# watsonyanghx/GAN_Lib_Tensorflow

Hardware: AMD Instinct MI355X
Metric: images/sec (G+D step) SNGAN-ResNet CIFAR-10 bs=64 (higher is better)
Workload: dtype bf16; 1 GPU; SNGAN ResNet CIFAR-10 32x32 bs=64 hinge: 1 G update (2x64 fakes) + 5 D updates (64 real + 64 fake) per step; global_batch=64, per_gpu_batch=64, parallelism=dp1, graphs=True, finite=True, collectives_in_graphs=False, grad_wire=fp32

## Files before the change

### gan_lib_tensorflow_amd/_lib.py

```python
import ctypes as C
import os

_HERE = os.path.dirname(os.path.abspath(__file__))
DTYPE = os.environ.get("GANK_DTYPE", "bf16").lower()
if DTYPE not in ("bf16", "fp16"):
    raise RuntimeError(f"GANK_DTYPE={DTYPE!r}: bf16 or fp16")
ACT_DTYPE_NAME = "bfloat16" if DTYPE == "bf16" else "float16"
LIB_PATH = os.path.join(_HERE, os.environ.get("GANK_LIB_NAME", "libgank.so" if DTYPE == "bf16" else "libgank_f16.so"))

P, I, L, F = C.c_void_p, C.c_int, C.c_long, C.c_float

IN_UPSAMPLE2X, IN_RELU, OUT_TANH, DY_UPSAMPLE2X, RES_UPSAMPLE2X, STATS_PREZEROED, OUT_POOLSUM2X = 1, 2, 4, 8, 64, 256, 512
STAT_SLOTS = 16


class SnDesc(C.Structure):
    _fields_ = [(n, P) for n in ("W", "u_in", "u_out", "v", "W_bar", "scal", "a", "b", "bpart",
                                 "dW_bar", "dW", "rowdot", "ga", "u_snap")] + \
               [("K", I), ("C", I), ("row_offset", I), ("chunk_offset", I)]


class WgradItem(C.Structure):
    _fields_ = [("x", P), ("dy", P), ("dw", P), ("dbias", P)]

# ... 8 lines not shown

class Res8Head(C.Structure):
    _fields_ = [("logits", P), ("head_w", P), ("pooled", P), ("loss", P), ("w_grad", P), ("b_grad", P), ("n_real", I), ("mode", I),
                ("loss_scale", F)]


class LabelDenseDesc(C.Structure):
    _fields_ = [("table", P), ("bias", P), ("out", P), ("V", I), ("D", I), ("weight", I)]


class CriticFeedDesc(C.Structure):
    _fields_ = [("real_all", P), ("labels_all", P), ("fake_all", P), ("both", P), ("labels2", P), ("slot", P), ("rng_state", P),
                ("done_counter", P), ("B", I), ("n_slots", I)]


PROTOTYPES = {
    "gank_version": [],
    "gank_act_dtype": [],
    "gank_last_error": [],
    "gank_conv2d_prep_weights": [P, P, P, I, I, I, P],
    "gank_conv2d_prep_weights_batched": [C.POINTER(PrepDesc), I, P],
    "gank_conv2d_fprop": [P, P, P, P, P, P, I, I, I, I, I, I, I, F, P],
    "gank_conv2d_fprop_stats": [P, P, P, P, P, P, I, I, I, I, I, I, I, F, P, I, P, P],
    "gank_conv2d_dgrad": [P, P, P, P, P, I, I, I, I, I, I, I, F, P],
    "gank_meanpool_conv1x1_fprop": [P, P, P, P, P, I, I, I, I, I, P],
    "gank_image_conv_pair_fprop": [P, P, P, P, P, P, P, P, I, I, I, I, I, P],
    "gank_conv2d_wgrad_batched": [C.POINTER(WgradItem), I, I, I, I, I, I, I, I, F, P],
    "gank_conv2d_wgrad_narrow_pair": [P, P, P, P, I, I, I, I, I, P, P, P, P, I, I, I, I, I, F, P],
    "gank_conv2d_wgrad_ws_elems": [I, I, I, I, I, I, I],
    "gank_conv1x1_wgrad_dgrad": [P, P, P, P, P, I, P, I, I, I, I, I, P],
    "gank_conv2d_wgrad": [P, P, P, P, P, L, I, I, I, I, I, I, I, F, P],
    "gank_upconv3x3_prep_weights": [P, P, P, I, I, P],
    "gank_upconv3x3_fprop": [P, P, P, P, P, I, I, I, I, I, I, P],
    "gank_upconv3x3_fprop_stats": [P, P, P, P, P, I, I, I, I, I, I, P, I, P, P],
    "gank_upconv3x3_dgrad": [P, P, P, P, I, I, I, I, I, P],
    "gank_convpool3x3_prep_weights": [P, P, P, I, I, P],
    "gank_convpool3x3_fprop": [P, P, P, P, P, I, I, I, I, I, I, P],
    "gank_convpool3x3_dgrad": [P, P, P, P, I, I, I, I, I, P],
    "gank_convpool3x3_wgrad": [P, P, P, P, P, L, I, I, I, I, I, I, P],
    "gank_convpool3x3_wgrad_ws_elems": [I, I, I, I, I],
    "gank_upconv3x3_wgrad_ws_elems": [I, I, I, I, I],
    "gank_upconv3x3_wgrad": [P, P, P, P, L, I, I, I, I, I, P],
    "gank_conv2d_general_fprop": [P, P, P, P, I, I, I, I, I, I, I, I, I, I, I, P],
    "gank_conv2d_general_dgrad": [P, P, P, P, I, I, I, I, I, I, I, I, I, P],
    "gank_conv2d_general_wgrad": [P, P, P, P, I, I, I, I, I, I, I, I, I, I, I, P],
    "gank_res8_chain_fwd": [P, P, P, P, P, P, I, I, I, P],
    "gank_res8_chain_bwd": [P, P, P, P, P, P, P, P, P, I, I, I, P],
    "gank_phase_stack4": [P, P, I, I, I, P],
    "gank_pad_rows": [P, P, C.c_long, I, I, I, I, P],
    "gank_tile_rows": [P, P, I, I, I, P],
    "gank_fewout_pack": [P, P, I, I, I, I, I, P],
    "gank_zero_f32": [P, C.c_long, P],
    "gank_img16_conv3x3": [P, P, P, P, P, P, I, I, I, I, P],
    "gank_cbn_relu_img16_conv3x3": [P, P, P, P, P, P, P, P, P, I, I, I, I, I, I, P, I, P],
    "gank_img16_conv3x3_stats": [P, P, P, P, P, P, I, I, I, I, P, I, P],
    "gank_res8_chain_fwd_head": [P, P, P, P, P, P, P, P, P, I, I, I, P],
    "gank_res8_chain_bwd_head": [C.POINTER(Res8Head), P, P, P, P, P, P, P, I, I, I, P],
    "gank_res8_conv3x3": [P, P, P, P, P, I, I, I, I, P, I, P],
    "gank_im2col_narrow": [P, P, I, I, I, I, I, I, I, I, I, I, P],
    "gank_tap_gather_up2": [P, P, P, I, I, I, I, I, I, I, I, P],
    "gank_tap_scatter_up2": [P, P, I, I, I, I, I, I, I, P],
    "gank_depth_to_space2": [P, P, I, I, I, I, P],
    "gank_space_to_depth2": [P, P, I, I, I, I, P],
    "gank_cpool_res_fprop": [P, P, P, P, P, I, I, I, I, I, I, P],
    "gank_cpool_res_dgrad": [P, P, P, P, I, I, I, I, I, P],
    "gank_cpool_res_dgrad_image_wgrad": [P, P, P, P, P, P, P, P, P, I, I, I, I, I, P, P],
# ... 161 lines not shown
```

### gan_lib_tensorflow_amd/csrc/conv_igemm.hip

```cpp
#include "gank_common.h"
#ifdef GANK_TUNING
static __device__ int gank_stats_dbg = 0;
static void gank_stats_dbg_init() {
  static const int v = gank_tune("GANK_STATS_DBG", 0);
  static bool done = false;
  if (!done) { done = true; if (v) (void)hipMemcpyToSymbol(HIP_SYMBOL(gank_stats_dbg), &v, sizeof(int)); }
}
#else
static inline void gank_stats_dbg_init() {}
#endif
#include <stdlib.h>
#include <type_traits>

#ifndef GANK_KMODE
#define GANK_KMODE 0
#endif
#define IG_IN_ZEROINS2X 16
#define IG_IN_STRIDE2 32
#define IG_RES_UP2X 128

struct IgemmArgs {
  const bf16* x;
  const bf16* w;
  const float* bias;
// ... 991 lines not shown
  gank_prof_tag(0, tag.c_str());
  hipLaunchKernelGGL((conv_narrow_in_kernel<KS, CIN, POOL>), dim3(a.tiles_m * a.tiles_n), dim3(256), 0, s, a);
  GANK_LAUNCH_OK("conv_narrow_in");
  return 0;
}

constexpr int PP_HALO_BYTES = 24576;
constexpr int PP_WSLOT_BYTES = 16384;
constexpr int PP_NSLOT = 6, PP_PD = 4;
constexpr int PP_WRING = 2 * PP_HALO_BYTES;
constexpr int PP_LDS_BYTES = PP_WRING + PP_NSLOT * PP_WSLOT_BYTES;

template <int N>
__device__ __forceinline__ void pp_wait_vmcnt() {
  static_assert(N == 0 || N == 4 || N == 6 || N == 7, "vmcnt value not instantiated");
  if constexpr (N == 0) asm volatile("s_waitcnt vmcnt(0)" ::: "memory");
  if constexpr (N == 4) asm volatile("s_waitcnt vmcnt(4)" ::: "memory");
  if constexpr (N == 6) asm volatile("s_waitcnt vmcnt(6)" ::: "memory");
  if constexpr (N == 7) asm volatile("s_waitcnt vmcnt(7)" ::: "memory");
}

#ifndef GANK_PP_M16
#define GANK_PP_M16 1
#endif
#ifdef GANK_ACT_F16
#define GANK_MFMA16(a, b, c) __builtin_amdgcn_mfma_f32_16x16x32_f16(a, b, c, 0, 0, 0)
#else
#define GANK_MFMA16(a, b, c) __builtin_amdgcn_mfma_f32_16x16x32_bf16(a, b, c, 0, 0, 0)
#endif
template <int MODE, int PW, bool STATS = false>
__global__ __launch_bounds__(512) void conv_igemm_pp_kernel(IgemmArgs a) {
  constexpr bool PHASE = (MODE & 4) != 0;
  constexpr int NT = PHASE ? 4 : 9;
  constexpr int PHH = 256 / PW;
  constexpr int HW_ = PW + 2, HROW = HW_ * 64;
  constexpr int HPX = (PHH + 2) * HW_;
  constexpr int RS = 32 / PW;
  constexpr int HSW = PW == 16 ? 1 : 2;
#if GANK_PP_M16
  auto pp_hswz = [](int hx) { return (hx >> 1) & 2; };
  auto pp_wswz = [](int co) { return (co >> 1) & 2; };
#else
  auto pp_hswz = [](int hx) { return (hx >> HSW) & 3; };
  auto pp_wswz = [](int co) { return (co >> 2) & 3; };
#endif
  static_assert(PW == 32 || PW == 16, "patch width");
  static_assert(HPX * 64 <= PP_HALO_BYTES, "halo image");
  extern __shared__ __attribute__((aligned(16))) char smem[];
  typedef __attribute__((address_space(3))) void* lds_t;
  const int tid = threadIdx.x, lane = tid & 63;
  const int wave = __builtin_amdgcn_readfirstlane(tid >> 6);
  const int wm = wave >> 2, wn = wave & 3;
  const int r = lane & 31, h = lane >> 5;
  const int prow = RS == 1 ? 0 : (r >> 4), pcol = RS == 1 ? r : (r & 15);

  const int nwg = a.tiles_m * a.tiles_n;
  const int lid = xcd_remap(blockIdx.x, nwg);
  const int tile_n = lid % a.tiles_n;
  int tile_m = lid / a.tiles_n;
  int phase = 0;
  if constexpr (PHASE) {
    if (a.phase_inner) { phase = tile_m & 3; tile_m >>= 2; }
    else { phase = tile_m / a.tiles_pp; tile_m -= phase * a.tiles_pp; }
  }
  const int pad_h = PHASE ? 1 - (phase >> 1) : 1, pad_w = PHASE ? 1 - (phase & 1) : 1;
  const int pw = a.W / PW, ph = a.H / PHH;
  const int n = tile_m / (pw * ph), pr = tile_m - n * pw * ph;
  const int py0 = (pr / pw) * PHH, px0 = (pr % pw) * PW;

  constexpr unsigned OOB = 0x7FFFFFF0u;
  const __amdgpu_buffer_rsrc_t rs_x = __builtin_amdgcn_make_buffer_rsrc(const_cast<bf16*>(a.x), 0, a.N * a.H * a.W * a.Cin * 2, 0x00020000);
  const __amdgpu_buffer_rsrc_t rs_w = __builtin_amdgcn_make_buffer_rsrc(const_cast<bf16*>(a.w) + (PHASE ? (long)phase * a.CoutPad * a.Kpad : 0L), 0,
                                                                        a.CoutPad * a.Kpad * 2, 0x00020000);

  unsigned h_off[6];
#pragma unroll
  for (int j = 0; j < 6; j++) {
    const int q = (j * 4 + wn) * 64 + lane;
    const int hp = q >> 2, hy = hp / HW_, hx = hp - hy * HW_;
    const int iy = py0 - 1 + hy, ix = px0 - 1 + hx;
    const bool ok = hp < HPX && (unsigned)iy < (unsigned)a.H && (unsigned)ix < (unsigned)a.W;
    h_off[j] = ok ? (unsigned)((((n * a.H + iy) * a.W + ix) * a.Cin + (((q & 3) ^ pp_hswz(hx)) << 3)) * 2) : OOB;
  }
  int w_off[2];
#pragma unroll
  for (int j = 0; j < 2; j++) {
    const int q = (j * 8 + wave) * 64 + lane;
    const int co = q >> 2;
    w_off[j] = ((tile_n * 256 + co) * a.Kpad + (((q & 3) ^ pp_wswz(co)) << 3)) * 2;
  }
  constexpr int ND = PHASE ? 2 : 3;
#if GANK_PP_M16
  const int p16 = lane & 15, kc = lane >> 4;
  constexpr int RPT = PW / 16;
  int a_lane, b_lane[ND];
  a_lane = PP_WRING + (wn * 64 + p16) * 64 + ((kc ^ pp_wswz(p16)) << 4);
#pragma unroll
  for (int d = 0; d < ND; d++) {
    const int hx = p16 + d + (PHASE ? 1 - pad_w : 0);
    const int hy = wm * (PHH / 2) + (PHASE ? 1 - pad_h : 0);
    b_lane[d] = hy * HROW + hx * 64 + ((kc ^ pp_hswz(hx)) << 4);
  }
#else
  int a_lane[2], b_lane[ND][2];
#pragma unroll
  for (int kk = 0; kk < 2; kk++) {
    a_lane[kk] = PP_WRING + (wn * 64 + r) * 64 + (((kk * 2 + h) ^ pp_wswz(r)) << 4);
#pragma unroll
    for (int d = 0; d < ND; d++) {
      const int hx = pcol + d + (PHASE ? 1 - pad_w : 0);
      const int hy = wm * (PHH / 2) + prow + (PHASE ? 1 - pad_h : 0);
      b_lane[d][kk] = hy * HROW + hx * 64 + (((kk * 2 + h) ^ pp_hswz(hx)) << 4);
    }
  }
#endif

  const int nch = a.Cin >> 5;
  auto issue_w = [&](int slot_bytes, int c, int tap) {
    const int koff = (tap * a.Cin + c * 32) * 2;
#pragma unroll
    for (int j = 0; j < 2; j++)
      __builtin_amdgcn_raw_ptr_buffer_load_lds(rs_w, (lds_t)(smem + PP_WRING + slot_bytes + (j * 8 + wave) * 1024), 16, w_off[j], koff, 0, 0);
  };
  auto issue_h = [&](int buf, int c, int j0) {
#pragma unroll
    for (int j = j0; j < j0 + 3; j++)
      __builtin_amdgcn_raw_ptr_buffer_load_lds(rs_x, (lds_t)(smem + buf * PP_HALO_BYTES + (j * 4 + wn) * 1024), 16, (int)(h_off[j] + (unsigned)c * 64u), 0, 0, 0);
  };

#if GANK_PP_M16
  f32x4 acc[4][8];
#pragma unroll
  for (int i = 0; i < 4; i++)
#pragma unroll
    for (int j = 0; j < 8; j++) acc[i][j] = f32x4{0.f, 0.f, 0.f, 0.f};
#else
  f32x16 acc[2][4];
#pragma unroll
  for (int i = 0; i < 2; i++)
#pragma unroll
    for (int j = 0; j < 4; j++)
#pragma unroll
      for (int e = 0; e < 16; e++) acc[i][j][e] = 0.f;
#endif

  if (wm == 1) { issue_h(0, 0, 0); issue_h(0, 0, 3); }
  {
    int c = 0, t = 0;
#pragma unroll
    for (int q = 0; q < PP_PD; q++) {
      issue_w(q * PP_WSLOT_BYTES, c, t);
      if (++t == NT) { t = 0; c++; }
      if (c >= nch) { c = nch - 1; t = NT - 1; }
    }
  }
  pp_wait_vmcnt<4>();
  __builtin_amdgcn_s_barrier();

  int rslot = 0, wslot = PP_PD * PP_WSLOT_BYTES;
  for (int c = 0; c < nch; c++) {
    const int hb = (c & 1) * PP_HALO_BYTES;
    const int cn = (c + 1 < nch) ? c + 1 : nch - 1;
    auto phase_step = [&](auto tc) {
      constexpr int t = decltype(tc)::value;
      constexpr int dh1 = PHASE ? t / 2 : t / 3, dw1 = PHASE ? t % 2 : t % 3;
      if (wm == 1) __builtin_amdgcn_s_barrier();
#if GANK_PP_M16
      bf16x8 fa[4], fb[8];
#pragma unroll
      for (int i = 0; i < 4; i++) fa[i] = *reinterpret_cast<const bf16x8*>(smem + rslot + i * 1024 + a_lane);
#pragma unroll
      for (int j = 0; j < 8; j++) fb[j] = *reinterpret_cast<const bf16x8*>(smem + hb + (j / RPT + dh1) * HROW + (j % RPT) * 1024 + b_lane[dw1]);
#else
      bf16x8 fa[2][2], fb[4][2];
#pragma unroll
      for (int kk = 0; kk < 2; kk++) {
#pragma unroll
        for (int i = 0; i < 2; i++) fa[i][kk] = *reinterpret_cast<const bf16x8*>(smem + rslot + i * 2048 + a_lane[kk]);
#pragma unroll
        for (int j = 0; j < 4; j++) fb[j][kk] = *reinterpret_cast<const bf16x8*>(smem + hb + (j * RS + dh1) * HROW + b_lane[dw1][kk]);
      }
#endif
      if constexpr (t < 2) { if (wm == 1) issue_h((c + 1) & 1, cn, 3 * t); }
      {
        constexpr int t4 = (t + PP_PD) % NT;
        int c4 = c + (t + PP_PD) / NT, tt = t4;
        if (c4 >= nch) { c4 = nch - 1; tt = NT - 1; }
        issue_w(wslot, c4, tt);
      }
      if constexpr (t < 2) { if (wm == 1) pp_wait_vmcnt<7>(); else pp_wait_vmcnt<4>(); }
      else pp_wait_vmcnt<4>();
      if (wm == 0) __builtin_amdgcn_s_barrier();
      asm volatile("s_waitcnt lgkmcnt(0)" ::: "memory");
#if GANK_PP_M16
      if constexpr ((MODE & 1) != 0) {
#pragma unroll
        for (int j = 0; j < 8; j++) fb[j] = __builtin_bit_cast(bf16x8, relu_bf16x8(__builtin_bit_cast(u32x4, fb[j])));
      }
      __builtin_amdgcn_sched_barrier(0);
#pragma unroll
      for (int i = 0; i < 4; i++)
#pragma unroll
        for (int j = 0; j < 8; j++)
          acc[i][j] = GANK_MFMA16(fa[i], fb[j], acc[i][j]);
#else
      if constexpr ((MODE & 1) != 0) {
#pragma unroll
        for (int j = 0; j < 4; j++)
#pragma unroll
          for (int kk = 0; kk < 2; kk++) fb[j][kk] = __builtin_bit_cast(bf16x8, relu_bf16x8(__builtin_bit_cast(u32x4, fb[j][kk])));
      }
      __builtin_amdgcn_sched_barrier(0);
#pragma unroll
      for (int kk = 0; kk < 2; kk++)
#pragma unroll
        for (int i = 0; i < 2; i++)
#pragma unroll
          for (int j = 0; j < 4; j++)
            acc[i][j] = GANK_MFMA32(fa[i][kk], fb[j][kk], acc[i][j]);
#endif
      __builtin_amdgcn_sched_barrier(0);
      rslot += PP_WSLOT_BYTES; if (rslot == PP_NSLOT * PP_WSLOT_BYTES) rslot = 0;
      wslot += PP_WSLOT_BYTES; if (wslot == PP_NSLOT * PP_WSLOT_BYTES) wslot = 0;
    };
    phase_step(std::integral_constant<int, 0>{}); phase_step(std::integral_constant<int, 1>{});
    phase_step(std::integral_constant<int, 2>{}); phase_step(std::integral_constant<int, 3>{});
    if constexpr (!PHASE) {
      phase_step(std::integral_constant<int, 4>{}); phase_step(std::integral_constant<int, 5>{}); phase_step(std::integral_constant<int, 6>{});
      phase_step(std::integral_constant<int, 7>{}); phase_step(std::integral_constant<int, 8>{});
    }
  }
  pp_wait_vmcnt<0>();

  const bool otanh = (a.flags & GANK_OUT_TANH) != 0;
  float keep1 = 0.f, keep2 = 0.f;
#if GANK_PP_M16
  {
    float st1[STATS ? 2 : 1][8], st2[STATS ? 2 : 1][8];
    if constexpr (STATS) {
#pragma unroll
      for (int P = 0; P < 2; P++)
#pragma unroll
        for (int e = 0; e < 8; e++) { st1[P][e] = 0.f; st2[P][e] = 0.f; }
    }
#pragma unroll
    for (int j = 0; j < 8; j++) {
      const int py = py0 + wm * (PHH / 2) + j / RPT, px = px0 + (j % RPT) * 16 + p16;
      const long m = PHASE ? ((long)(n * 2 * a.H + 2 * py + (phase >> 1))) * (2 * a.W) + 2 * px + (phase & 1) : ((long)(n * a.H + py)) * a.W + px;
      const long mr = (!PHASE && (a.flags & IG_RES_UP2X)) ? ((long)(n * (a.H >> 1) + (py >> 1))) * (a.W >> 1) + (px >> 1) : m;
      bf16x8 outl[2];
#pragma unroll
      for (int P = 0; P < 2; P++) {
        const int co = tile_n * 256 + wn * 64 + (2 * P + (kc & 1)) * 16 + 8 * (kc >> 1);
        float v[8];
#pragma unroll
        for (int e = 0; e < 4; e++) {
          float lo = acc[2 * P][j][e] * a.scale, hi = acc[2 * P + 1][j][e] * a.scale;
          asm volatile("s_nop 1\n\tv_permlane16_swap_b32 %0, %1" : "+v"(lo), "+v"(hi));
          v[e] = lo;
          v[4 + e] = hi;
        }
        const long o = m * a.Cout + co;
        float bb[8] = {0.f, 0.f, 0.f, 0.f, 0.f, 0.f, 0.f, 0.f}, d[8];
        if (a.bias) {
          const f32x4 b0 = *reinterpret_cast<const f32x4*>(a.bias + co), b1 = *reinterpret_cast<const f32x4*>(a.bias + co + 4);
#pragma unroll
          for (int e = 0; e < 4; e++) { bb[e] = b0[e]; bb[4 + e] = b1[e]; }
        }
#pragma unroll
        for (int e = 0; e < 8; e++) { d[e] = v[e]; v[e] += bb[e]; }
        if (a.mask) {
          const bf16x8 mk = *reinterpret_cast<const bf16x8*>(a.mask + o);
#pragma unroll
          for (int e = 0; e < 8; e++) { const bool on = bf2f(mk[e]) > 0.f; v[e] = on ? v[e] : 0.f; d[e] = on ? d[e] : -bb[e]; }
        }
        if (a.res) {
          const bf16x8 rs = *reinterpret_cast<const bf16x8*>(a.res + mr * a.Cout + co);
#pragma unroll
          for (int e = 0; e < 8; e++) { const float t = bf2f(rs[e]); v[e] += t; d[e] += t; }
        }
        if constexpr (STATS) {
#pragma unroll
          for (int e = 0; e < 8; e++) { st1[P][e] += d[e]; st2[P][e] += d[e] * d[e]; }
        }
#pragma unroll
        for (int e = 0; e < 8; e++) outl[P][e] = f2bf(otanh ? tanhf(v[e]) : v[e]);
      }
      bf16* line = a.y + m * a.Cout + tile_n * 256 + wn * 64 + (kc & 1) * 16 + 8 * (kc >> 1);
#pragma unroll
      for (int P = 0; P < 2; P++) *reinterpret_cast<bf16x8*>(line + 32 * P) = outl[P];
    }
    if constexpr (STATS) {
#pragma unroll
      for (int P = 0; P < 2; P++)
#pragma unroll
        for (int e = 0; e < 8; e++) {
          const float s1 = pp_row_sum(st1[P][e]), s2 = pp_row_sum(st2[P][e]);
          const bool mine = p16 == P * 8 + e;
          keep1 = mine ? s1 : keep1;
          keep2 = mine ? s2 : keep2;
        }
    }
  }
  if constexpr (STATS) {
    float* dst = a.stat_sums + ((long)(n / a.stat_n_per_group) * GANK_STAT_SLOTS + (blockIdx.x % GANK_STAT_SLOTS)) * 2 * a.Cout;
    const int co = tile_n * 256 + wn * 64 + (2 * (p16 >> 3) + (kc & 1)) * 16 + 8 * (kc >> 1) + (p16 & 7);
#ifdef GANK_TUNING
    if (gank_stats_dbg) return;
#endif
    atomicAdd(dst + co, keep1);
    atomicAdd(dst + a.Cout + co, keep2);
  }
#else
  {
    float st1[STATS ? 2 : 1][2][8], st2[STATS ? 2 : 1][2][8];
    if constexpr (STATS) {
#pragma unroll
      for (int i = 0; i < 2; i++)
#pragma unroll
        for (int q = 0; q < 2; q++)
#pragma unroll
          for (int e = 0; e < 8; e++) { st1[i][q][e] = 0.f; st2[i][q][e] = 0.f; }
    }
// ... 70 lines not shown
    const int ci = r >> 4, cq = (r >> 3) & 1, ce = r & 7;
    const int co = tile_n * 256 + (wn * 2 + ci) * 32 + 16 * cq + 8 * h + ce;
#ifdef GANK_TUNING
    if (gank_stats_dbg) return;
#endif
    atomicAdd(dst + co, keep1);
    atomicAdd(dst + a.Cout + co, keep2);
  }
#endif
}

static thread_local int tl_stats_done = 0;
__global__ void ig_zero_kernel(float* __restrict__ p, int n) {
  const int i = blockIdx.x * blockDim.x + threadIdx.x;
  if (i < n) p[i] = 0.f;
}

static void stats_zero(const IgemmArgs& a, hipStream_t s);
static int t128_min() {
  static const int v = gank_tune("GANK_IGEMM_T128_MIN", 192);
  return v;
}
static bool igemm_stats_ok(const IgemmArgs& a, int BM, int BN) {
  static const int env = gank_tune("GANK_IGEMM_STATS", 1);
  return env && a.stat_sums != nullptr && !(a.flags & GANK_OUT_TANH) && a.M % BM == 0 && a.Cout % BN == 0 &&
         ((long)a.stat_n_per_group * a.H * a.W) % BM == 0;
}
template <int MODE, int PW>
static int launch_pp(const IgemmArgs& a0, hipStream_t s) {
  IgemmArgs a = a0;
  const bool stats = a.stat_sums != nullptr;
  if (stats) { tl_stats_done = 1; stats_zero(a, s); }
  constexpr bool PHASE = (MODE & 4) != 0;
  const int tiles = a.N * (a.H / (256 / PW)) * (a.W / PW);
  a.tiles_pp = tiles;
  a.phase_inner = phase_inner_env();
  a.tiles_m = PHASE ? 4 * tiles : tiles;
  a.tiles_n = a.Cout / 256;
  if (PHASE) { a.Kpad = 4 * a.Cin; a.Hin = a.H; a.Win = a.W; }
  auto kern = stats ? conv_igemm_pp_kernel<MODE, PW, true> : conv_igemm_pp_kernel<MODE, PW, false>;
  if (stats) { GANK_MAX_DYNAMIC_LDS((conv_igemm_pp_kernel<MODE, PW, true>), PP_LDS_BYTES, "conv_igemm_pp"); }
  else { GANK_MAX_DYNAMIC_LDS((conv_igemm_pp_kernel<MODE, PW, false>), PP_LDS_BYTES, "conv_igemm_pp"); }
  static const std::string tag = gank_format("conv_igemm_pp_kernel<%d, %d>", MODE, PW);
  gank_prof_tag(0, tag.c_str());
  hipLaunchKernelGGL(kern, dim3(a.tiles_m * a.tiles_n), dim3(512), PP_LDS_BYTES, s, a);
  GANK_LAUNCH_OK("conv_igemm_pp");
  return 0;
}
static int pp_patch_width(int H, int W) { return (W % 32 == 0 && H % 8 == 0) ? 32 : (W % 16 == 0 && H % 16 == 0) ? 16 : 0; }
static int pp_env() {
  static const int v = gank_tune("GANK_IGEMM_PP", 2);
  return v;
}
static bool pp_enough_blocks(const IgemmArgs& a, int phases) {
  const int pw = pp_patch_width(a.H, a.W);
  return pw != 0 && (long)phases * a.N * (a.H / (256 / pw)) * (a.W / pw) * (a.Cout / 256) >= 224;
}
static bool pp_phase_ok(const IgemmArgs& a) {
  return pp_env() >= 2 && a.Cout % 256 == 0 && a.Cin % 32 == 0 && pp_enough_blocks(a, 4);
}
static int launch_pp_phase(const IgemmArgs& a, hipStream_t s) {
  const bool relu = (a.flags & GANK_IN_RELU) != 0;
  if (pp_patch_width(a.H, a.W) == 32) return relu ? launch_pp<5, 32>(a, s) : launch_pp<4, 32>(a, s);
  return relu ? launch_pp<5, 16>(a, s) : launch_pp<4, 16>(a, s);
}

template <int MODE, int BN>
static int launch_patch(const IgemmArgs& a0, hipStream_t s) {
  IgemmArgs a = a0;
  a.tiles_m = a.N * (a.H / 8) * (a.W / 16);
  a.tiles_n = a.CoutPad / BN;
  const size_t lds = ((size_t)10 * HROWP + (size_t)2 * BN * LROW) * sizeof(bf16);
  auto kern = conv_igemm_patch_kernel<MODE, BN>;
  GANK_MAX_DYNAMIC_LDS(kern, (int)lds, "conv_igemm_patch");
  static const std::string tag = gank_format("conv_igemm_patch_kernel<%d, %d>", MODE, BN);
  gank_prof_tag(0, tag.c_str());
  hipLaunchKernelGGL(kern, dim3(a.tiles_m * a.tiles_n), dim3(256), lds, s, a);
  GANK_LAUNCH_OK("conv_igemm_patch");
  return 0;
}

template <int WM, int WN, int TM, int TN, bool PACKED, int PF, int MODE>
static int launch_cfg(const IgemmArgs& a0, hipStream_t s) {
  IgemmArgs a = a0;
  constexpr int BM = WM * TM * 32, BN = WN * TN * 32;
  a.tiles_m = cdiv(a.M, BM);
  a.tiles_n = a.CoutPad / BN;
  const size_t lds = (size_t)2 * (BM + BN) * LROW * sizeof(bf16);
  static const std::string tag = gank_format("conv_igemm_kernel<%d, %d, %d, %d, %s, %d, %d>", WM, WN, TM, TN, PACKED ? "true" : "false", PF, MODE);
  gank_prof_tag(0, tag.c_str());
  if constexpr (!PACKED && MODE == 0 && TN * 16 <= 32) {
    if (igemm_stats_ok(a, BM, BN)) {
      auto kern = conv_igemm_kernel<WM, WN, TM, TN, PACKED, PF, MODE, true>;
      GANK_MAX_DYNAMIC_LDS(kern, (int)lds, "conv_igemm");
      tl_stats_done = 1;
// ... 260 lines not shown

extern "C" int gank_conv2d_general_fprop(const void* x, const void* wf, const float* bias, void* y, int N, int Hin, int Win,
                                         int Hout, int Wout, int Cin, int Cout, int ksize, int stride, int pad, int flags, void* stream) {
  GANK_REQUIRE(stride == 1 || stride == 2, "conv2d_general_fprop: stride %d (1 or 2)", stride);
  GANK_REQUIRE(pad >= 0 && pad < ksize, "conv2d_general_fprop: pad %d outside [0, ksize)", pad);
  GANK_REQUIRE(!((flags & GANK_IN_UPSAMPLE2X) && stride == 2), "conv2d_general_fprop: upsampled input with stride 2");
  GANK_REQUIRE(Hin > 0 && Win > 0 && Hout > 0 && Wout > 0, "conv2d_general_fprop: bad sizes");
  IgemmArgs a{};
  a.x = (const bf16*)x; a.w = (const bf16*)wf; a.bias = bias; a.y = (bf16*)y;
  a.N = N; a.H = Hout; a.W = Wout; a.Hin = Hin; a.Win = Win;
  a.Cin = Cin; a.Cout = Cout; a.ks = ksize; a.pad = pad;
  a.flags = (flags & (GANK_IN_UPSAMPLE2X | GANK_IN_RELU | GANK_OUT_TANH)) | (stride == 2 ? IG_IN_STRIDE2 : 0);
  a.scale = 1.f;
  return gank_igemm_dispatch(a, (hipStream_t)stream);
}
extern "C" int gank_conv2d_general_dgrad(const void* dy, const void* wd, const void* relu_ref, void* dx, int N, int Hx, int Wx,
                                         int Hdy, int Wdy, int Cin, int Cout, int ksize, int pad, void* stream) {
  GANK_REQUIRE(pad >= 0 && pad < ksize, "conv2d_general_dgrad: pad %d outside [0, ksize)", pad);
  IgemmArgs a{};
  a.x = (const bf16*)dy; a.w = (const bf16*)wd; a.mask = (const bf16*)relu_ref; a.y = (bf16*)dx;
  a.N = N; a.H = Hx; a.W = Wx; a.Hin = Hdy; a.Win = Wdy;
  a.Cin = Cout; a.Cout = Cin; a.ks = ksize; a.pad = ksize - 1 - pad;
  a.scale = 1.f;
  return gank_igemm_dispatch(a, (hipStream_t)stream);
}

static int upconv3x3_fprop_impl(const void* x, const void* wph, const float* bias, const void* residual, void* y,
                                int N, int Hl, int Wl, int Cin, int Cout, int flags, float* stat_sums, int groups, void* stream) {
  GANK_REQUIRE(Cin % 64 == 0, "upconv3x3_fprop: Cin must be a multiple of 64 (got %d)", Cin);
  IgemmArgs a{};
  a.x = (const bf16*)x; a.w = (const bf16*)wph; a.bias = bias; a.res = (const bf16*)residual; a.y = (bf16*)y;
  a.N = N; a.H = Hl; a.W = Wl; a.Hin = Hl; a.Win = Wl;
  a.Cin = Cin; a.Cout = Cout; a.ks = 2; a.pad = 0;
  a.flags = flags & GANK_OUT_TANH;
  a.scale = 1.f;
  hipStream_t s = (hipStream_t)stream;
  a.taps = 4; a.CoutPad = roundup(Cout, 32); a.Kpad = 4 * Cin; a.nsteps = a.Kpad / 64;
  a.M = N * Hl * Wl; a.sw = log2_or_neg(Wl); a.shw = log2_or_neg(Hl * Wl);
  GANK_REQUIRE((long)N * Hl * Wl * Cin < (1L << 30) && (long)a.M * 4 * Cout < (1L << 31), "upconv3x3_fprop: tensor too large");
  if (stats_setup(a, stat_sums, groups, N, Cout, s, flags)) return 1;
  gank_prof_begin(0, 2.0 * a.M * 4.0 * (double)Cout * 4 * Cin, s, 2.0 * ((double)a.M * Cin + 16.0 * Cin * Cout + 4.0 * a.M * Cout + (residual ? 4.0 * a.M * Cout : 0.0)));
  int rc;
  const long tiles128 = 4L * cdiv(a.M, 128) * (a.CoutPad / 128);
  if (pp_phase_ok(a)) rc = launch_pp_phase(a, s);
  else if (patch_phase_ok(a)) rc = launch_patch_phase<4>(a, s);
  else if (a.CoutPad % 128 == 0 && tiles128 >= t128_min()) rc = launch_phase<2, 2, 2, 2, 2>(a, s);
  else if (a.CoutPad % 64 == 0) rc = launch_phase<2, 2, 1, 1, 4>(a, s);
  else rc = launch_phase<4, 1, 2, 1, 2>(a, s);
  gank_prof_end(0, s);
  return rc;
}

extern "C" int gank_upconv3x3_fprop(const void* x, const void* wph, const float* bias, const void* residual, void* y,
                                    int N, int Hl, int Wl, int Cin, int Cout, int flags, void* stream) {
  return upconv3x3_fprop_impl(x, wph, bias, residual, y, N, Hl, Wl, Cin, Cout, flags, nullptr, 0, stream);
}
extern "C" int gank_upconv3x3_fprop_stats(const void* x, const void* wph, const float* bias, const void* residual, void* y,
                                          int N, int Hl, int Wl, int Cin, int Cout, int flags, float* stat_sums, int groups, int* produced,
                                          void* stream) {
  GANK_REQUIRE(stat_sums && produced, "upconv3x3_fprop_stats: null statistics pointers");
  const int rc = upconv3x3_fprop_impl(x, wph, bias, residual, y, N, Hl, Wl, Cin, Cout, flags, stat_sums, groups, stream);
  *produced = tl_stats_done;
  return rc;
}

extern "C" int gank_upconv3x3_dgrad(const void* dy, const void* wd4, const void* relu_ref, void* dx, int N, int Hl, int Wl,
                                    int Cin, int Cout, void* stream) {
  IgemmArgs a{};
  a.x = (const bf16*)dy; a.w = (const bf16*)wd4; a.mask = (const bf16*)relu_ref; a.y = (bf16*)dx;
  a.N = N; a.H = Hl; a.W = Wl; a.Hin = 2 * Hl; a.Win = 2 * Wl;
  a.Cin = Cout; a.Cout = Cin; a.ks = 4; a.pad = 1;
  a.flags = IG_IN_STRIDE2;
  a.scale = 1.f;
// ... 64 lines not shown
```

### gan_lib_tensorflow_amd/kernels.py

```python
import ctypes as C

import torch

from . import _lib
from ._lib import IN_UPSAMPLE2X, IN_RELU, OUT_TANH, DY_UPSAMPLE2X, RES_UPSAMPLE2X, STATS_PREZEROED, OUT_POOLSUM2X, SnDesc, PrepDesc, WgradItem, LabelDenseDesc, Res8Head, SlabJob

BF16, F32, I32 = getattr(torch, _lib.ACT_DTYPE_NAME), torch.float32, torch.int32


def _stream():
    return C.c_void_p(torch.cuda.current_stream().cuda_stream)


def _p(t, dtype=None, name="tensor"):
    if t is None:
        return None
    if not t.is_cuda:
        raise RuntimeError(f"gank: {name} must live on the GPU (no CPU path exists)")
    if not t.is_contiguous():
        raise RuntimeError(f"gank: {name} must be contiguous, got strides {t.stride()} for {tuple(t.shape)}")
    if dtype is not None and t.dtype != dtype:
        raise RuntimeError(f"gank: {name} must be {dtype}, got {t.dtype}")
    return C.c_void_p(t.data_ptr())

# ... 432 lines not shown
    _lib.check(lib().gank_conv2d_general_wgrad(_p(x, BF16, "x"), _p(dy, BF16, "dy"), _p(dw, F32, "dw"), _p(dbias, F32, "dbias"), n, hx, wx, hdy, wdy,
                                               cin, cout, ksize, stride, pad, flags, _stream()), "conv2d_general_wgrad")
    return dw


def upconv3x3_prep(w):
    _, _, cin, cout = w.shape
    old = getattr(w, "_prep_up", None)
    if old is not None:
        wph, wd4 = old
    else:
        wph = torch.empty((4, _roundup(cout, 32), 4 * cin), dtype=BF16, device=w.device)
        wd4 = torch.empty((_roundup(cin, 32), _roundup(16 * cout, 64)), dtype=BF16, device=w.device)
    _lib.check(lib().gank_upconv3x3_prep_weights(_p(w.detach(), F32, "w"), _p(wph), _p(wd4), cin, cout, _stream()), "upconv3x3_prep")
    w._prep_up = (wph, wd4)
    return wph, wd4


def upconv3x3_fprop(x, wph, bias, cout, flags=0, residual=None, stats_groups=0):
    n, hl, wl, cin = x.shape
    y = torch.empty((n, 2 * hl, 2 * wl, cout), dtype=BF16, device=x.device)
    if stats_groups:
        sums, pre = stats_arena.take((stats_groups, _lib.STAT_SLOTS, 2, cout), x.device)
        produced = C.c_int(0)
        _lib.check(lib().gank_upconv3x3_fprop_stats(_p(x, BF16, "x"), _p(wph, BF16), _p(bias, F32, "bias"), _p(residual, BF16, "residual"),
                                                    _p(y), n, hl, wl, cin, cout, flags | (STATS_PREZEROED if pre else 0), _p(sums), stats_groups, C.byref(produced), _stream()),
                   "upconv3x3_fprop_stats")
        return y, (ConvStats(sums, bias, stats_groups) if produced.value else None)
    _lib.check(lib().gank_upconv3x3_fprop(_p(x, BF16, "x"), _p(wph, BF16), _p(bias, F32, "bias"), _p(residual, BF16, "residual"),
                                          _p(y), n, hl, wl, cin, cout, flags, _stream()), "upconv3x3_fprop")
    return y


def upconv3x3_dgrad(dy, wd4, cin, relu_ref=None):
    n, h2, w2, cout = dy.shape
    dx = torch.empty((n, h2 // 2, w2 // 2, cin), dtype=BF16, device=dy.device)
    _lib.check(lib().gank_upconv3x3_dgrad(_p(dy, BF16, "dy"), _p(wd4, BF16), _p(relu_ref, BF16, "relu_ref"), _p(dx),
                                          n, h2 // 2, w2 // 2, cin, cout, _stream()), "upconv3x3_dgrad")
    return dx


def convpool3x3_prep(w):
    _, _, cin, cout = w.shape
    old = getattr(w, "_prep_pool", None)
    if old is not None:
        wp4, wphd = old
    else:
        wp4 = torch.empty((_roundup(cout, 32), _roundup(16 * cin, 64)), dtype=BF16, device=w.device)
        wphd = torch.empty((4, _roundup(cin, 32), 4 * cout), dtype=BF16, device=w.device)
    _lib.check(lib().gank_convpool3x3_prep_weights(_p(w.detach(), F32, "w"), _p(wp4), _p(wphd), cin, cout, _stream()), "convpool3x3_prep")
    w._prep_pool = (wp4, wphd)
    return wp4, wphd


def convpool3x3_fprop(x, wp4, bias, cout, flags=0, residual=None):
    n, h, w, cin = x.shape
    y = torch.empty((n, h // 2, w // 2, cout), dtype=BF16, device=x.device)
    _lib.check(lib().gank_convpool3x3_fprop(_p(x, BF16, "x"), _p(wp4, BF16), _p(bias, F32, "bias"), _p(residual, BF16, "residual"),
                                            _p(y), n, h // 2, w // 2, cin, cout, flags, _stream()), "convpool3x3_fprop")
    return y


def convpool3x3_dgrad(dy, wphd, cin, relu_ref=None):
    n, hp, wp, cout = dy.shape
    dx = torch.empty((n, 2 * hp, 2 * wp, cin), dtype=BF16, device=dy.device)
    _lib.check(lib().gank_convpool3x3_dgrad(_p(dy, BF16, "dy"), _p(wphd, BF16), _p(relu_ref, BF16, "relu_ref"), _p(dx),
# ... 1265 lines not shown
```

### include/gank.h

```cpp
#ifndef GANK_H
#define GANK_H

#include <stddef.h>
#include <stdint.h>

#ifdef __cplusplus
extern "C" {
#endif

#define GANK_VERSION 100

#define GANK_IN_UPSAMPLE2X 1
#define GANK_IN_RELU 2
#define GANK_OUT_TANH 4
#define GANK_DY_UPSAMPLE2X 8
#define GANK_STAT_SLOTS 16
#define GANK_STATS_PREZEROED 256
#define GANK_RES_UPSAMPLE2X 64
#define GANK_OUT_POOLSUM2X 512

int gank_version(void);
int gank_act_dtype(void);
const char* gank_last_error(void);

// ... 75 lines not shown
  const void* pooled;
  float* loss;
  float* w_grad;
  float* b_grad;
  int n_real, mode;
  float loss_scale;
} gank_res8_head;
int gank_res8_chain_fwd_head(const void* x, const void* const* w_rfrag, const float* const* bias, void* const* h1,
                             void* const* y, void* pooled, const float* head_w, const float* head_b, void* logits, int N, int C,
                             int nblocks, void* stream);
int gank_res8_chain_bwd_head(const gank_res8_head* head, const void* ylast, void* dy_out, const void* const* wd_rfrag,
                             const void* const* h1, const void* const* xin, void* const* g1, void* const* dx, int N, int C,
                             int nblocks, void* stream);

int gank_img16_conv3x3(const void* x, const void* w_rfrag, const float* bias, const void* relu_ref, const void* residual, void* y,
                       int N, int Cin, int Cout, int flags, void* stream);
int gank_cbn_relu_img16_conv3x3(const void* x, const int32_t* labels, const float* gamma, const float* beta, const float* stats,
                                const void* w_rfrag, const float* bias, const void* residual, void* y, int N, int Cin, int Cout,
                                int groups, int n_labels, int flags, float* stat_sums, int stat_groups, void* stream);
int gank_img16_conv3x3_stats(const void* x, const void* w_rfrag, const float* bias, const void* relu_ref, const void* residual, void* y,
                             int N, int Cin, int Cout, int flags, float* stat_sums, int stat_groups, void* stream);

int gank_res8_conv3x3(const void* x, const void* w_rfrag, const float* bias, const void* residual, void* y, int N, int Cin,
                      int Cout, int flags, float* stat_sums, int stat_groups, void* stream);

int gank_cpool_res_fprop(const void* x, const void* w_rfrag, const float* bias, const void* residual, void* y, int N, int Hp,
                         int Wp, int Cin, int Cout, int flags, void* stream);
int gank_cpool_res_dgrad(const void* dy, const void* w_rfrag, const void* relu_ref, void* dx, int N, int Hp, int Wp, int Cin,
                         int Cout, void* stream);
int gank_cpool_res_dgrad_image_wgrad(const void* dy, const void* w_rfrag, const void* relu_ref, const void* x_image, float* dw1,
                                     float* db1, const void* x_pooled, float* dws, float* dbs, int N, int Hp, int Wp, int Cin,
                                     int Cout, float* slabs, void* stream);

int gank_upconv3x3_prep_weights(const float* w, void* wph, void* wd4, int Cin, int Cout, void* stream);
int gank_upconv3x3_fprop(const void* x, const void* wph, const float* bias, const void* residual, void* y,
                         int N, int Hl, int Wl, int Cin, int Cout, int flags, void* stream);
int gank_upconv3x3_fprop_stats(const void* x, const void* wph, const float* bias, const void* residual, void* y,
                               int N, int Hl, int Wl, int Cin, int Cout, int flags, float* stat_sums, int groups, int* produced,
                               void* stream);
int gank_upconv3x3_dgrad(const void* dy, const void* wd4, const void* relu_ref, void* dx, int N, int Hl, int Wl,
                         int Cin, int Cout, void* stream);

int gank_convpool3x3_prep_weights(const float* w, void* wp4, void* wphd, int Cin, int Cout, void* stream);
int gank_convpool3x3_fprop(const void* x, const void* wp4, const float* bias, const void* residual, void* y,
                           int N, int Hp, int Wp, int Cin, int Cout, int flags, void* stream);
int gank_convpool3x3_dgrad(const void* dy, const void* wphd, const void* relu_ref, void* dx, int N, int Hp, int Wp,
                           int Cin, int Cout, void* stream);
long gank_upconv3x3_wgrad_ws_elems(int N, int H, int W, int Cin, int Cout);
int gank_upconv3x3_wgrad(const void* x_low, const void* dy, float* dw, float* ws16, long ws_elems, int N, int H, int W, int Cin, int Cout,
                         void* stream);
long gank_convpool3x3_wgrad_ws_elems(int N, int Hp, int Wp, int Cin, int Cout);
int gank_convpool3x3_wgrad(const void* x, const void* dy, float* dw, float* dbias, float* ws16, long ws_elems, int N, int Hp, int Wp,
                           int Cin, int Cout, int flags, void* stream);

int gank_conv2d_general_fprop(const void* x, const void* wf, const float* bias, void* y, int N, int Hin, int Win,
                              int Hout, int Wout, int Cin, int Cout, int ksize, int stride, int pad, int flags, void* stream);
int gank_conv2d_general_dgrad(const void* dy, const void* wd, const void* relu_ref, void* dx, int N, int Hx, int Wx,
                              int Hdy, int Wdy, int Cin, int Cout, int ksize, int pad, void* stream);
int gank_conv2d_general_wgrad(const void* x, const void* dy, float* dw, float* dbias, int N, int Hx, int Wx, int Hdy, int Wdy,
                              int Cin, int Cout, int ksize, int stride, int pad, int flags, void* stream);

int gank_meanpool_conv1x1_fprop(const void* x, const void* wf, const float* bias, void* y, void* pooled,
                                int N, int H, int W, int Cin, int Cout, void* stream);
int gank_image_conv_pair_fprop(const void* x, const void* wf1, const float* bias1, void* y1, const void* wfs, const float* biass, void* ys,
                               void* pooled, int N, int H, int W, int Cout1, int Couts, void* stream);

// ... 257 lines not shown
```

Measured before the change: 60170 images/sec.

## Add whole-image tiles to phase-mode upconv implicit GEMM for 4x4 and 8x8 inputs

```diff
diff --git a/gan_lib_tensorflow_amd/_lib.py b/gan_lib_tensorflow_amd/_lib.py
--- a/gan_lib_tensorflow_amd/_lib.py
+++ b/gan_lib_tensorflow_amd/_lib.py
@@ -64,6 +64,7 @@
     "gank_conv2d_wgrad": [P, P, P, P, P, L, I, I, I, I, I, I, I, F, P],
     "gank_upconv3x3_prep_weights": [P, P, P, I, I, P],
     "gank_upconv3x3_fprop": [P, P, P, P, P, I, I, I, I, I, I, P],
+    "gank_pp_whole_image": [I],
     "gank_upconv3x3_fprop_stats": [P, P, P, P, P, I, I, I, I, I, I, P, I, P, P],
     "gank_upconv3x3_dgrad": [P, P, P, P, I, I, I, I, I, P],
     "gank_convpool3x3_prep_weights": [P, P, P, I, I, P],
diff --git a/gan_lib_tensorflow_amd/csrc/conv_igemm.hip b/gan_lib_tensorflow_amd/csrc/conv_igemm.hip
--- a/gan_lib_tensorflow_amd/csrc/conv_igemm.hip
+++ b/gan_lib_tensorflow_amd/csrc/conv_igemm.hip
@@ -1047,19 +1047,25 @@
 __global__ __launch_bounds__(512) void conv_igemm_pp_kernel(IgemmArgs a) {
   constexpr bool PHASE = (MODE & 4) != 0;
   constexpr int NT = PHASE ? 4 : 9;
-  constexpr int PHH = 256 / PW;
+  constexpr bool WHOLE = PW <= 8;
+  constexpr int PIX = WHOLE ? 128 : 256;
+  constexpr int MT = PIX / 32;
+  constexpr int PHH = WHOLE ? PW : 256 / PW;
+  constexpr int IPT = WHOLE ? PIX / (PW * PW) : 1;
   constexpr int HW_ = PW + 2, HROW = HW_ * 64;
-  constexpr int HPX = (PHH + 2) * HW_;
+  constexpr int HPI = (PHH + 2) * HW_;
+  constexpr int HPX = IPT * HPI;
+  static_assert(!WHOLE || (PHASE && GANK_PP_M16), "whole-image tiles: phase mode, 16x16x32 fragments");
   constexpr int RS = 32 / PW;
   constexpr int HSW = PW == 16 ? 1 : 2;
 #if GANK_PP_M16
-  auto pp_hswz = [](int hx) { return (hx >> 1) & 2; };
+  auto pp_hswz = [](int hx) { return WHOLE ? (hx & 2) : ((hx >> 1) & 2); };
   auto pp_wswz = [](int co) { return (co >> 1) & 2; };
 #else
   auto pp_hswz = [](int hx) { return (hx >> HSW) & 3; };
   auto pp_wswz = [](int co) { return (co >> 2) & 3; };
 #endif
-  static_assert(PW == 32 || PW == 16, "patch width");
+  static_assert(PW == 32 || PW == 16 || PW == 8 || PW == 4, "patch width");
   static_assert(HPX * 64 <= PP_HALO_BYTES, "halo image");
   extern __shared__ __attribute__((aligned(16))) char smem[];
   typedef __attribute__((address_space(3))) void* lds_t;
@@ -1080,7 +1086,8 @@
   }
   const int pad_h = PHASE ? 1 - (phase >> 1) : 1, pad_w = PHASE ? 1 - (phase & 1) : 1;
   const int pw = a.W / PW, ph = a.H / PHH;
-  const int n = tile_m / (pw * ph), pr = tile_m - n * pw * ph;
+  const int n = WHOLE ? tile_m * IPT : tile_m / (pw * ph);
+  const int pr = WHOLE ? 0 : tile_m - n * pw * ph;
   const int py0 = (pr / pw) * PHH, px0 = (pr % pw) * PW;
 
   constexpr unsigned OOB = 0x7FFFFFF0u;
@@ -1092,10 +1099,10 @@
 #pragma unroll
   for (int j = 0; j < 6; j++) {
     const int q = (j * 4 + wn) * 64 + lane;
-    const int hp = q >> 2, hy = hp / HW_, hx = hp - hy * HW_;
+    const int hp = q >> 2, img = WHOLE ? hp / HPI : 0, hq = hp - img * HPI, hy = hq / HW_, hx = hq - hy * HW_;
     const int iy = py0 - 1 + hy, ix = px0 - 1 + hx;
-    const bool ok = hp < HPX && (unsigned)iy < (unsigned)a.H && (unsigned)ix < (unsigned)a.W;
-    h_off[j] = ok ? (unsigned)((((n * a.H + iy) * a.W + ix) * a.Cin + (((q & 3) ^ pp_hswz(hx)) << 3)) * 2) : OOB;
+    const bool ok = hp < HPX && n + img < a.N && (unsigned)iy < (unsigned)a.H && (unsigned)ix < (unsigned)a.W;
+    h_off[j] = ok ? (unsigned)(((((n + img) * a.H + iy) * a.W + ix) * a.Cin + (((q & 3) ^ pp_hswz(hx)) << 3)) * 2) : OOB;
   }
   int w_off[2];
 #pragma unroll
@@ -1107,15 +1114,23 @@
   constexpr int ND = PHASE ? 2 : 3;
 #if GANK_PP_M16
   const int p16 = lane & 15, kc = lane >> 4;
-  constexpr int RPT = PW / 16;
+  constexpr int RPT = WHOLE ? 1 : PW / 16;
   int a_lane, b_lane[ND];
   a_lane = PP_WRING + (wn * 64 + p16) * 64 + ((kc ^ pp_wswz(p16)) << 4);
 #pragma unroll
   for (int d = 0; d < ND; d++) {
-    const int hx = p16 + d + (PHASE ? 1 - pad_w : 0);
-    const int hy = wm * (PHH / 2) + (PHASE ? 1 - pad_h : 0);
-    b_lane[d] = hy * HROW + hx * 64 + ((kc ^ pp_hswz(hx)) << 4);
-  }
+    if constexpr (WHOLE) {
+      const int hx = p16 % PW + d + 1 - pad_w, hy = p16 / PW + 1 - pad_h;
+      b_lane[d] = (wm * (IPT / 2) * HPI + hy * HW_ + hx) * 64 + ((kc ^ pp_hswz(hx)) << 4);
+    } else {
+      const int hx = p16 + d + (PHASE ? 1 - pad_w : 0);
+      const int hy = wm * (PHH / 2) + (PHASE ? 1 - pad_h : 0);
+      b_lane[d] = hy * HROW + hx * 64 + ((kc ^ pp_hswz(hx)) << 4);
+    }
+  }
+  auto pp_tile_off = [](int j) {
+    return WHOLE ? ((j * 16) / (PW * PW)) * HPI * 64 + (((j * 16) % (PW * PW)) / PW) * HROW : (j / RPT) * HROW + (j % RPT) * 1024;
+  };
 #else
   int a_lane[2], b_lane[ND][2];
 #pragma unroll
@@ -1144,11 +1159,11 @@
   };
 
 #if GANK_PP_M16
-  f32x4 acc[4][8];
+  f32x4 acc[4][MT];
 #pragma unroll
   for (int i = 0; i < 4; i++)
 #pragma unroll
-    for (int j = 0; j < 8; j++) acc[i][j] = f32x4{0.f, 0.f, 0.f, 0.f};
+    for (int j = 0; j < MT; j++) acc[i][j] = f32x4{0.f, 0.f, 0.f, 0.f};
 #else
   f32x16 acc[2][4];
 #pragma unroll
@@ -1181,11 +1196,11 @@
       constexpr int dh1 = PHASE ? t / 2 : t / 3, dw1 = PHASE ? t % 2 : t % 3;
       if (wm == 1) __builtin_amdgcn_s_barrier();
 #if GANK_PP_M16
-      bf16x8 fa[4], fb[8];
+      bf16x8 fa[4], fb[MT];
 #pragma unroll
       for (int i = 0; i < 4; i++) fa[i] = *reinterpret_cast<const bf16x8*>(smem + rslot + i * 1024 + a_lane);
 #pragma unroll
-      for (int j = 0; j < 8; j++) fb[j] = *reinterpret_cast<const bf16x8*>(smem + hb + (j / RPT + dh1) * HROW + (j % RPT) * 1024 + b_lane[dw1]);
+      for (int j = 0; j < MT; j++) fb[j] = *reinterpret_cast<const bf16x8*>(smem + hb + dh1 * HROW + pp_tile_off(j) + b_lane[dw1]);
 #else
       bf16x8 fa[2][2], fb[4][2];
 #pragma unroll
@@ -1210,13 +1225,13 @@
 #if GANK_PP_M16
       if constexpr ((MODE & 1) != 0) {
 #pragma unroll
-        for (int j = 0; j < 8; j++) fb[j] = __builtin_bit_cast(bf16x8, relu_bf16x8(__builtin_bit_cast(u32x4, fb[j])));
+        for (int j = 0; j < MT; j++) fb[j] = __builtin_bit_cast(bf16x8, relu_bf16x8(__builtin_bit_cast(u32x4, fb[j])));
       }
       __builtin_amdgcn_sched_barrier(0);
 #pragma unroll
       for (int i = 0; i < 4; i++)
 #pragma unroll
-        for (int j = 0; j < 8; j++)
+        for (int j = 0; j < MT; j++)
           acc[i][j] = GANK_MFMA16(fa[i], fb[j], acc[i][j]);
 #else
       if constexpr ((MODE & 1) != 0) {
@@ -1259,10 +1274,14 @@
         for (int e = 0; e < 8; e++) { st1[P][e] = 0.f; st2[P][e] = 0.f; }
     }
 #pragma unroll
-    for (int j = 0; j < 8; j++) {
-      const int py = py0 + wm * (PHH / 2) + j / RPT, px = px0 + (j % RPT) * 16 + p16;
-      const long m = PHASE ? ((long)(n * 2 * a.H + 2 * py + (phase >> 1))) * (2 * a.W) + 2 * px + (phase & 1) : ((long)(n * a.H + py)) * a.W + px;
-      const long mr = (!PHASE && (a.flags & IG_RES_UP2X)) ? ((long)(n * (a.H >> 1) + (py >> 1))) * (a.W >> 1) + (px >> 1) : m;
+    for (int j = 0; j < MT; j++) {
+      const int wp = wm * (PIX / 2) + j * 16 + p16;
+      const int nn = WHOLE ? n + wp / (PW * PW) : n;
+      const bool valid = !WHOLE || nn < a.N;
+      const int py = WHOLE ? (wp % (PW * PW)) / PW : py0 + wm * (PHH / 2) + j / RPT;
+      const int px = WHOLE ? wp % PW : px0 + (j % RPT) * 16 + p16;
+      const long m = PHASE ? ((long)(nn * 2 * a.H + 2 * py + (phase >> 1))) * (2 * a.W) + 2 * px + (phase & 1) : ((long)(nn * a.H + py)) * a.W + px;
+      const long mr = (!PHASE && (a.flags & IG_RES_UP2X)) ? ((long)(nn * (a.H >> 1) + (py >> 1))) * (a.W >> 1) + (px >> 1) : m;
       bf16x8 outl[2];
 #pragma unroll
       for (int P = 0; P < 2; P++) {
@@ -1284,26 +1303,26 @@
         }
 #pragma unroll
         for (int e = 0; e < 8; e++) { d[e] = v[e]; v[e] += bb[e]; }
-        if (a.mask) {
+        if (a.mask && valid) {
           const bf16x8 mk = *reinterpret_cast<const bf16x8*>(a.mask + o);
 #pragma unroll
           for (int e = 0; e < 8; e++) { const bool on = bf2f(mk[e]) > 0.f; v[e] = on ? v[e] : 0.f; d[e] = on ? d[e] : -bb[e]; }
         }
-        if (a.res) {
+        if (a.res && valid) {
           const bf16x8 rs = *reinterpret_cast<const bf16x8*>(a.res + mr * a.Cout + co);
 #pragma unroll
           for (int e = 0; e < 8; e++) { const float t = bf2f(rs[e]); v[e] += t; d[e] += t; }
         }
         if constexpr (STATS) {
 #pragma unroll
-          for (int e = 0; e < 8; e++) { st1[P][e] += d[e]; st2[P][e] += d[e] * d[e]; }
+          for (int e = 0; e < 8; e++) { const float dv = valid ? d[e] : 0.f; st1[P][e] += dv; st2[P][e] += dv * dv; }
         }
 #pragma unroll
         for (int e = 0; e < 8; e++) outl[P][e] = f2bf(otanh ? tanhf(v[e]) : v[e]);
       }
       bf16* line = a.y + m * a.Cout + tile_n * 256 + wn * 64 + (kc & 1) * 16 + 8 * (kc >> 1);
 #pragma unroll
-      for (int P = 0; P < 2; P++) *reinterpret_cast<bf16x8*>(line + 32 * P) = outl[P];
+      for (int P = 0; P < 2; P++) if (valid) *reinterpret_cast<bf16x8*>(line + 32 * P) = outl[P];
     }
     if constexpr (STATS) {
 #pragma unroll
@@ -1440,7 +1459,7 @@
   const bool stats = a.stat_sums != nullptr;
   if (stats) { tl_stats_done = 1; stats_zero(a, s); }
   constexpr bool PHASE = (MODE & 4) != 0;
-  const int tiles = a.N * (a.H / (256 / PW)) * (a.W / PW);
+  const int tiles = PW <= 8 ? cdiv(a.N, 128 / (PW * PW)) : a.N * (a.H / (256 / PW)) * (a.W / PW);
   a.tiles_pp = tiles;
   a.phase_inner = phase_inner_env();
   a.tiles_m = PHASE ? 4 * tiles : tiles;
@@ -1464,11 +1483,40 @@
   const int pw = pp_patch_width(a.H, a.W);
   return pw != 0 && (long)phases * a.N * (a.H / (256 / pw)) * (a.W / pw) * (a.Cout / 256) >= 224;
 }
+static std::atomic<int> g_pp_whole{-1};
+static int pp_whole_mode() {
+  int v = g_pp_whole.load(std::memory_order_relaxed);
+  if (v < 0) { v = gank_tune("GANK_IGEMM_PP_WHOLE", 1); g_pp_whole.store(v, std::memory_order_relaxed); }
+  return v;
+}
+extern "C" int gank_pp_whole_image(int mode) {
+  const int old = pp_whole_mode();
+  if (mode >= 0) g_pp_whole.store(mode > 2 ? 2 : mode, std::memory_order_relaxed);
+  return old;
+}
+static int pp_whole_width(const IgemmArgs& a) {
+#if GANK_PP_M16
+  const int mode = pp_whole_mode();
+  if (!mode || a.H != a.W || (a.H != 8 && a.H != 4)) return 0;
+  const int ipt = 128 / (a.H * a.W);
+  if (a.stat_sums && a.stat_groups > 1 && a.stat_n_per_group % ipt != 0) return 0;
+  const long blocks = 4L * cdiv(a.N, ipt) * (a.Cout / 256);
+  if (mode < 2 && blocks < (a.H == 4 ? 160 : 224)) return 0;
+  return a.H;
+#else
+  (void)a;
+  return 0;
+#endif
+}
 static bool pp_phase_ok(const IgemmArgs& a) {
-  return pp_env() >= 2 && a.Cout % 256 == 0 && a.Cin % 32 == 0 && pp_enough_blocks(a, 4);
+  return pp_env() >= 2 && a.Cout % 256 == 0 && a.Cin % 32 == 0 && (pp_enough_blocks(a, 4) || pp_whole_width(a) != 0);
 }
 static int launch_pp_phase(const IgemmArgs& a, hipStream_t s) {
   const bool relu = (a.flags & GANK_IN_RELU) != 0;
+#if GANK_PP_M16
+  if (pp_whole_width(a) == 8) return relu ? launch_pp<5, 8>(a, s) : launch_pp<4, 8>(a, s);
+  if (pp_whole_width(a) == 4) return relu ? launch_pp<5, 4>(a, s) : launch_pp<4, 4>(a, s);
+#endif
   if (pp_patch_width(a.H, a.W) == 32) return relu ? launch_pp<5, 32>(a, s) : launch_pp<4, 32>(a, s);
   return relu ? launch_pp<5, 16>(a, s) : launch_pp<4, 16>(a, s);
 }
@@ -1795,13 +1843,14 @@
   a.x = (const bf16*)x; a.w = (const bf16*)wph; a.bias = bias; a.res = (const bf16*)residual; a.y = (bf16*)y;
   a.N = N; a.H = Hl; a.W = Wl; a.Hin = Hl; a.Win = Wl;
   a.Cin = Cin; a.Cout = Cout; a.ks = 2; a.pad = 0;
-  a.flags = flags & GANK_OUT_TANH;
+  a.flags = flags & (GANK_OUT_TANH | GANK_IN_RELU);
   a.scale = 1.f;
   hipStream_t s = (hipStream_t)stream;
   a.taps = 4; a.CoutPad = roundup(Cout, 32); a.Kpad = 4 * Cin; a.nsteps = a.Kpad / 64;
   a.M = N * Hl * Wl; a.sw = log2_or_neg(Wl); a.shw = log2_or_neg(Hl * Wl);
   GANK_REQUIRE((long)N * Hl * Wl * Cin < (1L << 30) && (long)a.M * 4 * Cout < (1L << 31), "upconv3x3_fprop: tensor too large");
   if (stats_setup(a, stat_sums, groups, N, Cout, s, flags)) return 1;
+  GANK_REQUIRE(!(a.flags & GANK_IN_RELU) || pp_phase_ok(a), "upconv3x3_fprop: GANK_IN_RELU needs a shape the two-group kernel takes");
   gank_prof_begin(0, 2.0 * a.M * 4.0 * (double)Cout * 4 * Cin, s, 2.0 * ((double)a.M * Cin + 16.0 * Cin * Cout + 4.0 * a.M * Cout + (residual ? 4.0 * a.M * Cout : 0.0)));
   int rc;
   const long tiles128 = 4L * cdiv(a.M, 128) * (a.CoutPad / 128);
diff --git a/gan_lib_tensorflow_amd/kernels.py b/gan_lib_tensorflow_amd/kernels.py
--- a/gan_lib_tensorflow_amd/kernels.py
+++ b/gan_lib_tensorflow_amd/kernels.py
@@ -488,6 +488,10 @@
     return y
 
 
+def pp_whole_image(mode):
+    return int(lib().gank_pp_whole_image(int(mode)))
+
+
 def upconv3x3_dgrad(dy, wd4, cin, relu_ref=None):
     n, h2, w2, cout = dy.shape
     dx = torch.empty((n, h2 // 2, w2 // 2, cin), dtype=BF16, device=dy.device)
diff --git a/include/gank.h b/include/gank.h
--- a/include/gank.h
+++ b/include/gank.h
@@ -131,6 +131,7 @@
                                      float* db1, const void* x_pooled, float* dws, float* dbs, int N, int Hp, int Wp, int Cin,
                                      int Cout, float* slabs, void* stream);
 
+int gank_pp_whole_image(int mode);
 int gank_upconv3x3_prep_weights(const float* w, void* wph, void* wd4, int Cin, int Cout, void* stream);
 int gank_upconv3x3_fprop(const void* x, const void* wph, const float* bias, const void* residual, void* y,
                          int N, int Hl, int Wl, int Cin, int Cout, int flags, void* stream);
```

Result: no change. 60470 images/sec (median of 6 runs) (+0.5%).
